# amisr/volumetricinterp

Hardware: AMD Instinct MI355X
Metric: fit+eval timesteps/sec (higher is better)
Workload: dtype f64

## Files before the change

volumetricinterp_amd/csrc/vi_walk.hip:

```cpp
#include "vi_common.h"
#include "vi_solver.h"

namespace {

using v4f64 = __attribute__((__vector_size__(4 * sizeof(double)))) double;

template <int NT, bool RES, int KL, bool PAD>
__global__ __launch_bounds__(NT * 64) void k_walk_rotate(int N, const double* __restrict__ AWA, const int* __restrict__ rec,
                                                         const double* __restrict__ V, const double* __restrict__ D2,
                                                         const int* __restrict__ basis, const double* __restrict__ y,
                                                         const double* __restrict__ alpha, double* __restrict__ X,
                                                         double* __restrict__ scl, double* __restrict__ yt)
{
    constexpr int KS = 4 * NT;
    constexpr int UNR = RES ? NT : 1;
    __shared__ double shV[KS * 64];
    __shared__ double shW[KS * 64];
    __shared__ double shB[KL > 0 ? NT * KL * 64 : 1];
    __shared__ double red[NT];
    const int64_t i = blockIdx.x;
    const int tid = threadIdx.x, lane = tid & 63, w = tid >> 6;
    const int n = lane & 15, g = lane >> 4;
    const int64_t NN = (int64_t)N * N;
    const double* Ai = AWA + (int64_t)rec[i] * NN;
    const double* Vi = V + (int64_t)basis[i] * NN;
    const double* D2i = D2 + (int64_t)basis[i] * NN;
    const double* yi = y + (int64_t)rec[i] * N;
    double* Xi = X + i * NN;
    const double a = alpha[i];
    const int c = 16 * w + n;
    const bool cok = c < N;

    const int cc = (!PAD || cok) ? c : N - 1;
    auto loadA = [&](int u) {
        const int k = 4 * u + g;
        if (!PAD) return Ai[(int64_t)k * N + c];
        return Ai[(int64_t)(k < N ? k : N - 1) * N + cc] * ((cok && k < N) ? 1.0 : 0.0);
    };
    auto loadV = [&](int blk, int u) {
        const int r = 16 * blk + n, k = 4 * u + g;
        if (!PAD) return Vi[(int64_t)r * N + k];
        return Vi[(int64_t)(r < N ? r : N - 1) * N + (k < N ? k : N - 1)] * ((r < N && k < N) ? 1.0 : 0.0);
    };
    for (int k = w; k < N; k += NT) {
        double acc = 0.0;
        for (int r = lane; r < N; r += 64) acc = fma(Vi[(int64_t)k * N + r], yi[r], acc);
        for (int o = 32; o > 0; o >>= 1) acc += __shfl_down(acc, o);
        if (lane == 0) yt[i * N + k] = acc;
    }

    constexpr int KR = KS - KL;
    double bA[RES ? KS : 1], bV[RES ? KR : 1];
    if (RES) {
#pragma unroll
        for (int u = 0; u < KS; ++u) bA[u] = loadA(u);
#pragma unroll
        for (int u = 0; u < KR; ++u) bV[u] = loadV(w, u);
#pragma unroll
        for (int u = KR; u < KS; ++u) shB[(w * KL + u - KR) * 64 + lane] = loadV(w, u);
    }
    auto getV = [&](int u) { return !RES ? loadV(w, u) : u < KR ? bV[u] : shB[(w * KL + u - KR) * 64 + lane]; };

    double mx = 0.0;
    for (int I = 0; I < NT; ++I) {
        if (RES) {
            if (w == I) {
#pragma unroll
                for (int u = 0; u < KS; ++u) shV[u * 64 + lane] = getV(u);
            }
        } else {
            for (int u = w; u < KS; u += NT) shV[u * 64 + lane] = loadV(I, u);
        }
        __syncthreads();
        v4f64 t = {0.0, 0.0, 0.0, 0.0};
#pragma unroll UNR
        for (int u0 = 0; u0 < KS; u0 += 4) {
            double av[4];
#pragma unroll
            for (int u = 0; u < 4; ++u) av[u] = shV[(u0 + u) * 64 + lane];
#pragma unroll
            for (int u = 0; u < 4; ++u)
                t = __builtin_amdgcn_mfma_f64_16x16x4f64(av[u], RES ? bA[u0 + u] : loadA(u0 + u), t, 0, 0, 0);
            __builtin_amdgcn_sched_barrier(0);
        }
#pragma unroll
        for (int r = 0; r < 4; ++r) shW[(4 * w + (n >> 2)) * 64 + (g + 4 * r) + 16 * (n & 3)] = t[r];
        __syncthreads();
        if (w <= I) {
            double d2v[4];
#pragma unroll
            for (int r = 0; r < 4; ++r) {
                const int row = 16 * I + g + 4 * r;
                d2v[r] = (!PAD || (cok && row < N)) ? D2i[(int64_t)row * N + c] : 0.0;
            }
            v4f64 d = {0.0, 0.0, 0.0, 0.0};
#pragma unroll UNR
            for (int u0 = 0; u0 < KS; u0 += 4) {
                double av[4];
#pragma unroll
                for (int u = 0; u < 4; ++u) av[u] = shW[(u0 + u) * 64 + lane];
#pragma unroll
                for (int u = 0; u < 4; ++u)
                    d = __builtin_amdgcn_mfma_f64_16x16x4f64(av[u], getV(u0 + u), d, 0, 0, 0);
                __builtin_amdgcn_sched_barrier(0);
            }
#pragma unroll
            for (int r = 0; r < 4; ++r) {
                const int row = 16 * I + g + 4 * r;
                if (!PAD || (cok && row < N)) {
                    const double v = fma(a, d2v[r], d[r]);
                    mx = fmax(mx, fabs(v));
                    Xi[(int64_t)row * N + c] = v;
                }
            }
        }
    }

    for (int o = 32; o > 0; o >>= 1) mx = fmax(mx, __shfl_xor(mx, o));
    if (lane == 0) red[w] = mx;
    __syncthreads();
    mx = 0.0;
#pragma unroll
    for (int q = 0; q < NT; ++q) mx = fmax(mx, red[q]);
    int ex = 0;
    double f = 1.0;
    if (mx > 0.0 && mx < 1.7e308) {
        (void)frexp(mx, &ex);
        f = ldexp(1.0, 1 - ex);
    }
    constexpr int RB = 8, CG = (16 * NT + 63) / 64;
    for (int r0 = w; r0 < N; r0 += RB * NT) {
        double xv[RB][CG];
#pragma unroll
        for (int q = 0; q < RB; ++q) {
            const int row = r0 + q * NT < N ? r0 + q * NT : N - 1;
            const int lim = 16 * (row / 16 + 1) < N ? 16 * (row / 16 + 1) : N;
#pragma unroll
            for (int m = 0; m < CG; ++m) {
                const int col = lane + 64 * m;
                xv[q][m] = Xi[(int64_t)row * N + (col < lim ? col : lim - 1)];
            }
        }
#pragma unroll
        for (int q = 0; q < RB; ++q) {
            const int row = r0 + q * NT;
            const int lim = 16 * (row / 16 + 1) < N ? 16 * (row / 16 + 1) : N;
#pragma unroll
            for (int m = 0; m < CG; ++m) {
                const int col = lane + 64 * m;
                if (row < N && col < lim) Xi[(int64_t)row * N + col] = xv[q][m] * f;
            }
        }
    }
    if (tid == 0) scl[i] = 1.0 / f;
}

template <int NT, bool RES, int KL, bool RESP>
void launch_walk_rotate(vi_ctx* c, int64_t B, int N, const double* AWA, const int* rec, const double* V, const double* D2,
                        const int* basis, const double* y, const double* alpha, double* X, double* scl, double* yt)
{
    if (N == 16 * NT)
        hipLaunchKernelGGL((k_walk_rotate<NT, RES, KL, false>), dim3((unsigned)B), dim3(NT * 64), 0, c->stream, N, AWA, rec, V, D2,
                           basis, y, alpha, X, scl, yt);
    else
        hipLaunchKernelGGL((k_walk_rotate<NT, RESP, 0, true>), dim3((unsigned)B), dim3(NT * 64), 0, c->stream, N, AWA, rec, V, D2,
                           basis, y, alpha, X, scl, yt);
}

}

int vi_walk_rotate(vi_ctx* c, int64_t B, int N, const double* d_AWA, const int* d_rec, const double* d_V, const double* d_D2,
                   const int* d_basis, const double* d_y, const double* d_alpha, double* d_X, double* d_scl, double* d_yt)
{
#define VI_W(NT, RES, KL, RESP)                                                                                                \
    case NT:                                                                                                          \
        launch_walk_rotate<NT, RES, KL, RESP>(c, B, N, d_AWA, d_rec, d_V, d_D2, d_basis, d_y, d_alpha, d_X, d_scl, d_yt);       \
        break
    switch ((N + 15) / 16) {
        VI_W(1, true, 0, true);
        VI_W(2, true, 0, true);
        VI_W(3, true, 0, true);
        VI_W(4, true, 0, true);
        VI_W(5, true, 0, true);
        VI_W(6, true, 0, true);
        VI_W(7, true, 0, true);
        VI_W(8, true, 0, true);
        VI_W(9, true, 16, false);
        VI_W(10, false, 0, false);
        VI_W(11, false, 0, false);
        VI_W(12, false, 0, false);
        VI_W(13, false, 0, false);
    default:
        vi_set_error("vi_walk_rotate: N=%d outside 1..208", N);
        return VI_ERR_UNSUPPORTED;
    }
#undef VI_W
    VI_HIP(hipGetLastError());
    return VI_OK;
}
```

Baseline: 3669.

## Process runs of systems per block, reusing held basis V operands

Each block now walks a run of S consecutive systems (default 4) rather than one. It keeps the basis matrix V fragments in registers and shared memory, reloading only when the basis index changes. The yt = V·y matvec is restructured to batch row loads into registers before reducing. Compile-time cycle-stamp instrumentation is added behind VI_STAMPS. The trade-offs are fewer blocks (less parallelism), a larger shared footprint from extra KL, and serialized per-system work inside each block.

```diff
diff --git a/volumetricinterp_amd/csrc/vi_walk.hip b/volumetricinterp_amd/csrc/vi_walk.hip
--- a/volumetricinterp_amd/csrc/vi_walk.hip
+++ b/volumetricinterp_amd/csrc/vi_walk.hip
@@ -1,12 +1,31 @@
 #include "vi_common.h"
 #include "vi_solver.h"
 
+#include <cstring>
+
+#ifdef VI_STAMPS
+__device__ unsigned long long g_walk_phases[16];
+#define WK_STAMP(k)                                                                   \
+    do {                                                                              \
+        const unsigned long long t_ = __builtin_readcyclecounter();                   \
+        if (threadIdx.x == 0) atomicAdd(&g_walk_phases[k], t_ - stamp_t);             \
+        stamp_t = __builtin_readcyclecounter();                                       \
+    } while (0)
+#define WK_COUNT(k) do { if (threadIdx.x == 0) atomicAdd(&g_walk_phases[k], 1ull); } while (0)
+#define WK_DRAIN() asm volatile("s_waitcnt vmcnt(0) lgkmcnt(0)" ::: "memory")
+#else
+#define WK_STAMP(k)
+#define WK_COUNT(k)
+#define WK_DRAIN()
+#endif
+
 namespace {
 
 using v4f64 = __attribute__((__vector_size__(4 * sizeof(double)))) double;
 
-template <int NT, bool RES, int KL, bool PAD>
-__global__ __launch_bounds__(NT * 64) void k_walk_rotate(int N, const double* __restrict__ AWA, const int* __restrict__ rec,
+template <int NT, bool RES, int KL, bool PAD, bool RUN>
+__global__ __launch_bounds__(NT * 64) void k_walk_rotate(int64_t B, int S, int N_, const double* __restrict__ AWA,
+                                                         const int* __restrict__ rec,
                                                          const double* __restrict__ V, const double* __restrict__ D2,
                                                          const int* __restrict__ basis, const double* __restrict__ y,
                                                          const double* __restrict__ alpha, double* __restrict__ X,
@@ -18,141 +37,214 @@
     __shared__ double shW[KS * 64];
     __shared__ double shB[KL > 0 ? NT * KL * 64 : 1];
     __shared__ double red[NT];
-    const int64_t i = blockIdx.x;
-    const int tid = threadIdx.x, lane = tid & 63, w = tid >> 6;
-    const int n = lane & 15, g = lane >> 4;
-    const int64_t NN = (int64_t)N * N;
-    const double* Ai = AWA + (int64_t)rec[i] * NN;
-    const double* Vi = V + (int64_t)basis[i] * NN;
-    const double* D2i = D2 + (int64_t)basis[i] * NN;
-    const double* yi = y + (int64_t)rec[i] * N;
-    double* Xi = X + i * NN;
-    const double a = alpha[i];
-    const int c = 16 * w + n;
-    const bool cok = c < N;
-
-    const int cc = (!PAD || cok) ? c : N - 1;
-    auto loadA = [&](int u) {
-        const int k = 4 * u + g;
-        if (!PAD) return Ai[(int64_t)k * N + c];
-        return Ai[(int64_t)(k < N ? k : N - 1) * N + cc] * ((cok && k < N) ? 1.0 : 0.0);
-    };
-    auto loadV = [&](int blk, int u) {
-        const int r = 16 * blk + n, k = 4 * u + g;
-        if (!PAD) return Vi[(int64_t)r * N + k];
-        return Vi[(int64_t)(r < N ? r : N - 1) * N + (k < N ? k : N - 1)] * ((r < N && k < N) ? 1.0 : 0.0);
-    };
-    for (int k = w; k < N; k += NT) {
-        double acc = 0.0;
-        for (int r = lane; r < N; r += 64) acc = fma(Vi[(int64_t)k * N + r], yi[r], acc);
-        for (int o = 32; o > 0; o >>= 1) acc += __shfl_down(acc, o);
-        if (lane == 0) yt[i * N + k] = acc;
-    }
-
+    static_assert(RES || !RUN, "a run of systems keeps bV: the variants that hold their operands only");
     constexpr int KR = KS - KL;
-    double bA[RES ? KS : 1], bV[RES ? KR : 1];
-    if (RES) {
-#pragma unroll
-        for (int u = 0; u < KS; ++u) bA[u] = loadA(u);
-#pragma unroll
-        for (int u = 0; u < KR; ++u) bV[u] = loadV(w, u);
-#pragma unroll
-        for (int u = KR; u < KS; ++u) shB[(w * KL + u - KR) * 64 + lane] = loadV(w, u);
-    }
-    auto getV = [&](int u) { return !RES ? loadV(w, u) : u < KR ? bV[u] : shB[(w * KL + u - KR) * 64 + lane]; };
-
-    double mx = 0.0;
-    for (int I = 0; I < NT; ++I) {
+    double bV[RES ? KR : 1];
+    int held = -1;
+    const int64_t i0 = RUN ? (int64_t)blockIdx.x * S : (int64_t)blockIdx.x;
+    const int64_t i1 = RUN ? (i0 + S < B ? i0 + S : B) : i0 + 1;
+#ifdef VI_STAMPS
+    unsigned long long stamp_t = __builtin_readcyclecounter();
+#endif
+    for (int64_t i = i0; i < i1; ++i) {
+        int N = N_, tid = threadIdx.x;
+        if (RUN) asm volatile("" : "+s"(N), "+v"(tid));
+        const int lane = tid & 63, w = tid >> 6;
+        const int n = lane & 15, g = lane >> 4;
+        const int64_t NN = (int64_t)N * N;
+        const int c = 16 * w + n;
+        const bool cok = c < N;
+        const int bi = RUN ? __builtin_amdgcn_readfirstlane(basis[i]) : basis[i];
+        const double* Ai = AWA + (int64_t)rec[i] * NN;
+        const double* Vi = V + (int64_t)bi * NN;
+        const double* D2i = D2 + (int64_t)bi * NN;
+        const double* yi = y + (int64_t)rec[i] * N;
+        double* Xi = X + i * NN;
+        const double a = alpha[i];
+
+        const int cc = (!PAD || cok) ? c : N - 1;
+        auto loadA = [&](int u) {
+            const int k = 4 * u + g;
+            if (!PAD) return Ai[(int64_t)k * N + c];
+            return Ai[(int64_t)(k < N ? k : N - 1) * N + cc] * ((cok && k < N) ? 1.0 : 0.0);
+        };
+        auto loadV = [&](int blk, int u) {
+            const int r = 16 * blk + n, k = 4 * u + g;
+            if (!PAD) return Vi[(int64_t)r * N + k];
+            return Vi[(int64_t)(r < N ? r : N - 1) * N + (k < N ? k : N - 1)] * ((r < N && k < N) ? 1.0 : 0.0);
+        };
+        constexpr int YB = 8, YR = (16 * NT + 63) / 64;
+        double yv[YR];
+#pragma unroll
+        for (int m = 0; m < YR; ++m) yv[m] = yi[lane + 64 * m < N ? lane + 64 * m : N - 1];
+        for (int k0 = w; k0 < N; k0 += YB * NT) {
+            double vv[YB][YR];
+#pragma unroll
+            for (int q = 0; q < YB; ++q) {
+                const int k = k0 + q * NT < N ? k0 + q * NT : N - 1;
+#pragma unroll
+                for (int m = 0; m < YR; ++m) vv[q][m] = Vi[(int64_t)k * N + (lane + 64 * m < N ? lane + 64 * m : N - 1)];
+            }
+#pragma unroll
+            for (int q = 0; q < YB; ++q) {
+                double acc = 0.0;
+#pragma unroll
+                for (int m = 0; m < YR; ++m)
+                    if (lane + 64 * m < N) acc = fma(vv[q][m], yv[m], acc);
+                for (int o = 32; o > 0; o >>= 1) acc += __shfl_down(acc, o);
+                if (lane == 0 && k0 + q * NT < N) yt[i * N + k0 + q * NT] = acc;
+            }
+        }
+        WK_DRAIN();
+        WK_STAMP(0);
+
+        double bA[RES ? KS : 1];
         if (RES) {
-            if (w == I) {
-#pragma unroll
-                for (int u = 0; u < KS; ++u) shV[u * 64 + lane] = getV(u);
-            }
-        } else {
-            for (int u = w; u < KS; u += NT) shV[u * 64 + lane] = loadV(I, u);
-        }
-        __syncthreads();
-        v4f64 t = {0.0, 0.0, 0.0, 0.0};
-#pragma unroll UNR
-        for (int u0 = 0; u0 < KS; u0 += 4) {
-            double av[4];
-#pragma unroll
-            for (int u = 0; u < 4; ++u) av[u] = shV[(u0 + u) * 64 + lane];
-#pragma unroll
-            for (int u = 0; u < 4; ++u)
-                t = __builtin_amdgcn_mfma_f64_16x16x4f64(av[u], RES ? bA[u0 + u] : loadA(u0 + u), t, 0, 0, 0);
-            __builtin_amdgcn_sched_barrier(0);
-        }
-#pragma unroll
-        for (int r = 0; r < 4; ++r) shW[(4 * w + (n >> 2)) * 64 + (g + 4 * r) + 16 * (n & 3)] = t[r];
-        __syncthreads();
-        if (w <= I) {
-            double d2v[4];
-#pragma unroll
-            for (int r = 0; r < 4; ++r) {
-                const int row = 16 * I + g + 4 * r;
-                d2v[r] = (!PAD || (cok && row < N)) ? D2i[(int64_t)row * N + c] : 0.0;
-            }
-            v4f64 d = {0.0, 0.0, 0.0, 0.0};
+#pragma unroll
+            for (int u = 0; u < KS; ++u) bA[u] = loadA(u);
+            WK_DRAIN();
+            WK_STAMP(1);
+            if (!RUN || bi != held) {
+#pragma unroll
+                for (int u = 0; u < KR; ++u) bV[u] = loadV(w, u);
+#pragma unroll
+                for (int u = KR; u < KS; ++u) shB[(w * KL + u - KR) * 64 + lane] = loadV(w, u);
+                held = bi;
+                WK_COUNT(11);
+            }
+            WK_DRAIN();
+            WK_STAMP(2);
+        }
+        auto getV = [&](int u) { return !RES ? loadV(w, u) : u < KR ? bV[u] : shB[(w * KL + u - KR) * 64 + lane]; };
+
+        double mx = 0.0;
+        for (int I = 0; I < NT; ++I) {
+            if (RES) {
+                if (w == I) {
+#pragma unroll
+                    for (int u = 0; u < (RUN ? KR : KS); ++u) shV[u * 64 + lane] = getV(u);
+                }
+            } else {
+                for (int u = w; u < KS; u += NT) shV[u * 64 + lane] = loadV(I, u);
+            }
+            WK_STAMP(3);
+            __syncthreads();
+            WK_STAMP(4);
+            v4f64 t = {0.0, 0.0, 0.0, 0.0};
 #pragma unroll UNR
             for (int u0 = 0; u0 < KS; u0 += 4) {
                 double av[4];
 #pragma unroll
-                for (int u = 0; u < 4; ++u) av[u] = shW[(u0 + u) * 64 + lane];
-#pragma unroll
                 for (int u = 0; u < 4; ++u)
-                    d = __builtin_amdgcn_mfma_f64_16x16x4f64(av[u], getV(u0 + u), d, 0, 0, 0);
+                    av[u] = RUN && u0 + u >= KR ? shB[(I * KL + u0 + u - KR) * 64 + lane] : shV[(u0 + u) * 64 + lane];
+#pragma unroll
+                for (int u = 0; u < 4; ++u)
+                    t = __builtin_amdgcn_mfma_f64_16x16x4f64(av[u], RES ? bA[u0 + u] : loadA(u0 + u), t, 0, 0, 0);
                 __builtin_amdgcn_sched_barrier(0);
             }
 #pragma unroll
-            for (int r = 0; r < 4; ++r) {
-                const int row = 16 * I + g + 4 * r;
-                if (!PAD || (cok && row < N)) {
-                    const double v = fma(a, d2v[r], d[r]);
-                    mx = fmax(mx, fabs(v));
-                    Xi[(int64_t)row * N + c] = v;
-                }
-            }
-        }
+            for (int r = 0; r < 4; ++r) shW[(4 * w + (n >> 2)) * 64 + (g + 4 * r) + 16 * (n & 3)] = t[r];
+            WK_STAMP(5);
+            __syncthreads();
+            WK_STAMP(6);
+            if (w <= I) {
+                double d2v[4];
+#pragma unroll
+                for (int r = 0; r < 4; ++r) {
+                    const int row = 16 * I + g + 4 * r;
+                    d2v[r] = (!PAD || (cok && row < N)) ? D2i[(int64_t)row * N + c] : 0.0;
+                }
+                v4f64 d = {0.0, 0.0, 0.0, 0.0};
+#pragma unroll UNR
+                for (int u0 = 0; u0 < KS; u0 += 4) {
+                    double av[4];
+#pragma unroll
+                    for (int u = 0; u < 4; ++u) av[u] = shW[(u0 + u) * 64 + lane];
+#pragma unroll
+                    for (int u = 0; u < 4; ++u)
+                        d = __builtin_amdgcn_mfma_f64_16x16x4f64(av[u], getV(u0 + u), d, 0, 0, 0);
+                    __builtin_amdgcn_sched_barrier(0);
+                }
+#pragma unroll
+                for (int r = 0; r < 4; ++r) {
+                    const int row = 16 * I + g + 4 * r;
+                    if (!PAD || (cok && row < N)) {
+                        const double v = fma(a, d2v[r], d[r]);
+                        mx = fmax(mx, fabs(v));
+                        Xi[(int64_t)row * N + c] = v;
+                    }
+                }
+            }
+            WK_STAMP(7);
+        }
+
+        for (int o = 32; o > 0; o >>= 1) mx = fmax(mx, __shfl_xor(mx, o));
+        if (lane == 0) red[w] = mx;
+        __syncthreads();
+        WK_STAMP(8);
+        mx = 0.0;
+#pragma unroll
+        for (int q = 0; q < NT; ++q) mx = fmax(mx, red[q]);
+        int ex = 0;
+        double f = 1.0;
+        if (mx > 0.0 && mx < 1.7e308) {
+            (void)frexp(mx, &ex);
+            f = ldexp(1.0, 1 - ex);
+        }
+        constexpr int RB = 8, CG = (16 * NT + 63) / 64;
+        for (int r0 = w; r0 < N; r0 += RB * NT) {
+            double xv[RB][CG];
+#pragma unroll
+            for (int q = 0; q < RB; ++q) {
+                const int row = r0 + q * NT < N ? r0 + q * NT : N - 1;
+                const int lim = 16 * (row / 16 + 1) < N ? 16 * (row / 16 + 1) : N;
+#pragma unroll
+                for (int m = 0; m < CG; ++m) {
+                    const int col = lane + 64 * m;
+                    xv[q][m] = Xi[(int64_t)row * N + (col < lim ? col : lim - 1)];
+                }
+            }
+#pragma unroll
+            for (int q = 0; q < RB; ++q) {
+                const int row = r0 + q * NT;
+                const int lim = 16 * (row / 16 + 1) < N ? 16 * (row / 16 + 1) : N;
+#pragma unroll
+                for (int m = 0; m < CG; ++m) {
+                    const int col = lane + 64 * m;
+                    if (row < N && col < lim) Xi[(int64_t)row * N + col] = xv[q][m] * f;
+                }
+            }
+        }
+        if (tid == 0) scl[i] = 1.0 / f;
+        WK_DRAIN();
+        WK_STAMP(9);
+        WK_COUNT(10);
     }
-
-    for (int o = 32; o > 0; o >>= 1) mx = fmax(mx, __shfl_xor(mx, o));
-    if (lane == 0) red[w] = mx;
-    __syncthreads();
-    mx = 0.0;
-#pragma unroll
-    for (int q = 0; q < NT; ++q) mx = fmax(mx, red[q]);
-    int ex = 0;
-    double f = 1.0;
-    if (mx > 0.0 && mx < 1.7e308) {
-        (void)frexp(mx, &ex);
-        f = ldexp(1.0, 1 - ex);
+}
+
+constexpr int WALK_RUN = 4;
+constexpr int WALK_RUN_KL = 4;
+int walk_run()
+{
+    static const int v = vi_env_is("VINTERP_WALK_FORM", "system") ? 1 : vi_env_int("VINTERP_WALK_RUN", WALK_RUN);
+    return v;
+}
+
+template <int NT, bool RES, int KL, bool PAD>
+void launch_walk_variant(vi_ctx* c, int64_t B, int N, const double* AWA, const int* rec, const double* V, const double* D2,
+                         const int* basis, const double* y, const double* alpha, double* X, double* scl, double* yt)
+{
+    const int S = walk_run();
+    if constexpr (RES) {
+        if (S > 1) {
+            constexpr int KLR = KL ? KL + WALK_RUN_KL : 0;
+            hipLaunchKernelGGL((k_walk_rotate<NT, RES, KLR, PAD, true>), dim3((unsigned)((B + S - 1) / S)), dim3(NT * 64), 0,
+                               c->stream, B, S, N, AWA, rec, V, D2, basis, y, alpha, X, scl, yt);
+            return;
+        }
     }
-    constexpr int RB = 8, CG = (16 * NT + 63) / 64;
-    for (int r0 = w; r0 < N; r0 += RB * NT) {
-        double xv[RB][CG];
-#pragma unroll
-        for (int q = 0; q < RB; ++q) {
-            const int row = r0 + q * NT < N ? r0 + q * NT : N - 1;
-            const int lim = 16 * (row / 16 + 1) < N ? 16 * (row / 16 + 1) : N;
-#pragma unroll
-            for (int m = 0; m < CG; ++m) {
-                const int col = lane + 64 * m;
-                xv[q][m] = Xi[(int64_t)row * N + (col < lim ? col : lim - 1)];
-            }
-        }
-#pragma unroll
-        for (int q = 0; q < RB; ++q) {
-            const int row = r0 + q * NT;
-            const int lim = 16 * (row / 16 + 1) < N ? 16 * (row / 16 + 1) : N;
-#pragma unroll
-            for (int m = 0; m < CG; ++m) {
-                const int col = lane + 64 * m;
-                if (row < N && col < lim) Xi[(int64_t)row * N + col] = xv[q][m] * f;
-            }
-        }
-    }
-    if (tid == 0) scl[i] = 1.0 / f;
+    hipLaunchKernelGGL((k_walk_rotate<NT, RES, KL, PAD, false>), dim3((unsigned)B), dim3(NT * 64), 0, c->stream, B, 1, N, AWA,
+                       rec, V, D2, basis, y, alpha, X, scl, yt);
 }
 
 template <int NT, bool RES, int KL, bool RESP>
@@ -160,11 +252,9 @@
                         const int* basis, const double* y, const double* alpha, double* X, double* scl, double* yt)
 {
     if (N == 16 * NT)
-        hipLaunchKernelGGL((k_walk_rotate<NT, RES, KL, false>), dim3((unsigned)B), dim3(NT * 64), 0, c->stream, N, AWA, rec, V, D2,
-                           basis, y, alpha, X, scl, yt);
+        launch_walk_variant<NT, RES, KL, false>(c, B, N, AWA, rec, V, D2, basis, y, alpha, X, scl, yt);
     else
-        hipLaunchKernelGGL((k_walk_rotate<NT, RESP, 0, true>), dim3((unsigned)B), dim3(NT * 64), 0, c->stream, N, AWA, rec, V, D2,
-                           basis, y, alpha, X, scl, yt);
+        launch_walk_variant<NT, RESP, 0, true>(c, B, N, AWA, rec, V, D2, basis, y, alpha, X, scl, yt);
 }
 
 }
@@ -198,3 +288,17 @@
     VI_HIP(hipGetLastError());
     return VI_OK;
 }
+
+#ifdef VI_STAMPS
+extern "C" int vi_debug_walk_phases(double* out, int reset)
+{
+    unsigned long long h[16];
+    if (hipMemcpyFromSymbol(h, HIP_SYMBOL(g_walk_phases), sizeof(h)) != hipSuccess) return -1;
+    for (int i = 0; i < 16; ++i) out[i] = (double)h[i];
+    if (reset) {
+        memset(h, 0, sizeof(h));
+        if (hipMemcpyToSymbol(HIP_SYMBOL(g_walk_phases), h, sizeof(h)) != hipSuccess) return -1;
+    }
+    return 0;
+}
+#endif
```

Result: no change. 3672, median of 2 (+0.1%).
